# levia-than/neptune-pde-solver

Hardware: AMD Instinct MI355X
Metric: stencil-cell-updates/s (higher is better)
Workload: dtype f64

## Files before the change

### neptune-pde-solver_amd/csrc/kernels/apply_march.hpp

```cpp
#pragma once
#include "apply_common.hpp"

namespace neptune_hip {

struct InView {
  int64_t plane_b;
  int32_t row_b;
  int32_t sh[3];
  int32_t lo[3], hi[3];
  int32_t fix_k, fix_d;
};

template <class T, int NIN>
struct MarchParams {
  const T* in[NIN];
  T* out;
  int32_t N0, N1, N2;
  InView view[NIN];
  int32_t Ks, Kl;
  int32_t plb[3], pub[3];
  int64_t olb[3];
  int32_t rI0, rI1;
  int32_t rJ0, rJ1;
  int32_t chunk;
  uint32_t nJ, nK;
};

template <class T, int NIN>
__device__ __forceinline__ uint32_t view_row_bytes(const MarchParams<T, NIN>& P, int n, int32_t j) {
  if (NIN > 1 && n > 0) {
    const InView& vw = P.view[n];
    j = j < vw.lo[1] ? vw.lo[1] : (j > vw.hi[1] ? vw.hi[1] : j);
    return (uint32_t)(j + vw.sh[1]) * (uint32_t)vw.row_b + (uint32_t)vw.sh[2] * (uint32_t)sizeof(T);
  }
  j = j < 0 ? 0 : (j >= P.N1 ? P.N1 - 1 : j);
  return (uint32_t)j * (uint32_t)P.N2 * (uint32_t)sizeof(T);
}
template <class T, int NIN>
__device__ __forceinline__ uint32_t view_cell_bytes(const MarchParams<T, NIN>& P, int n, int32_t k) {
  if (NIN > 1 && n > 0) {
    const InView& vw = P.view[n];
    k = k < vw.lo[2] ? vw.lo[2] : (k > vw.hi[2] ? vw.hi[2] : k);
  } else {
    k = k < 0 ? 0 : (k >= P.N2 ? P.N2 - 1 : k);
  }
  return (uint32_t)k * (uint32_t)sizeof(T);
}
template <class T, int NIN>
__device__ __forceinline__ uint32_t view_lane_bytes(const MarchParams<T, NIN>& P, int n, int32_t k) {
  constexpr int VK = 16 / (int)sizeof(T);
  int32_t kmax = P.Kl;
  if (NIN > 1 && n > 0) kmax = P.view[n].hi[2] - VK + 1;
  return (uint32_t)(k < kmax ? k : kmax) * (uint32_t)sizeof(T);
}
template <class T, int NIN>
__device__ __forceinline__ const char* view_plane_base(const MarchParams<T, NIN>& P, int n, int32_t ip) {
  if (NIN > 1 && n > 0) {
    const InView& vw = P.view[n];
    const int32_t ic = ip < vw.lo[0] ? vw.lo[0] : (ip > vw.hi[0] ? vw.hi[0] : ip);
    return reinterpret_cast<const char*>(P.in[n]) + (int64_t)(ic + vw.sh[0]) * vw.plane_b;
  }
  const int32_t ic = ip < 0 ? 0 : (ip >= P.N0 ? P.N0 - 1 : ip);
  return reinterpret_cast<const char*>(P.in[n]) + (int64_t)ic * ((int64_t)P.N1 * P.N2 * (int64_t)sizeof(T));
}

template <class T> struct Vec16;
template <> struct Vec16<double> { typedef double type __attribute__((ext_vector_type(2))); };
template <> struct Vec16<float> { typedef float type __attribute__((ext_vector_type(4))); };

template <class T>
__device__ __forceinline__ typename Vec16<T>::type view_fix(typename Vec16<T>::type v, bool star, int32_t d) {
  if (d != 0) {
    if constexpr (sizeof(T) == 8) {
      v[0] = star ? v[1] : v[0];
    } else {
      if (d & 1) { const bool c = star; typename Vec16<T>::type w = v; v[0] = c ? w[1] : w[0]; v[1] = c ? w[2] : w[1]; v[2] = c ? w[3] : w[2]; }
      if (d & 2) { const bool c = star; typename Vec16<T>::type w = v; v[0] = c ? w[2] : w[0]; v[1] = c ? w[3] : w[1]; }
    }
  }
  return v;
}
template <class T, int NIN>
__device__ __forceinline__ int32_t view_fix_d(const MarchParams<T, NIN>& P, int n) { return (NIN > 1 && n > 0) ? P.view[n].fix_d : 0; }
template <class T, int NIN>
__device__ __forceinline__ bool view_fix_star(const MarchParams<T, NIN>& P, int n, int32_t k) { return NIN > 1 && n > 0 && k == P.view[n].fix_k; }

template <bool DPP>
__device__ __forceinline__ int shift32_from_prev(int x, int edge, int lane) {
  if constexpr (DPP) {
    return __builtin_amdgcn_update_dpp(edge, x, 0x138, 0xf, 0xf, false);
  } else {
    const int s = __shfl_up(x, 1);
    return lane == 0 ? edge : s;
  }
}
template <bool DPP>
__device__ __forceinline__ int shift32_from_next(int x, int edge, int lane) {
  if constexpr (DPP) {
    return __builtin_amdgcn_update_dpp(edge, x, 0x130, 0xf, 0xf, false);
  } else {
    const int s = __shfl_down(x, 1);
    return lane == kWave - 1 ? edge : s;
  }
}
template <bool DPP>
__device__ __forceinline__ float from_prev(float x, float edge, int lane) {
  return __int_as_float(shift32_from_prev<DPP>(__float_as_int(x), __float_as_int(edge), lane));
}
template <bool DPP>
__device__ __forceinline__ float from_next(float x, float edge, int lane) {
  return __int_as_float(shift32_from_next<DPP>(__float_as_int(x), __float_as_int(edge), lane));
}
template <bool DPP>
__device__ __forceinline__ double from_prev(double x, double edge, int lane) {
  const int lo = shift32_from_prev<DPP>(__double2loint(x), __double2loint(edge), lane);
  const int hi = shift32_from_prev<DPP>(__double2hiint(x), __double2hiint(edge), lane);
  return __hiloint2double(hi, lo);
}
template <bool DPP>
__device__ __forceinline__ double from_next(double x, double edge, int lane) {
  const int lo = shift32_from_next<DPP>(__double2loint(x), __double2loint(edge), lane);
  const int hi = shift32_from_next<DPP>(__double2hiint(x), __double2hiint(edge), lane);
  return __hiloint2double(hi, lo);
}

template <class T>
__device__ __forceinline__ T scalar_load(const T* p) {
  typedef const __attribute__((address_space(4))) T* cptr;
  return *(cptr)(p);
}

template <class T, int RANK, int NIN, class FP, int RJ, int r, int e, bool JK = false>
struct MarchAcc {
  static constexpr int VK = 16 / sizeof(T);
  static constexpr int R0 = JK ? 0 : FP::R0, R1 = JK ? FP::R0 : FP::R1, R2 = FP::R2;
  static constexpr unsigned HMASK = FP::HALO_MASK;
  static constexpr int NH = popcount_u(HMASK), NHX = NH ? NH : 1;
  static constexpr int NP = 2 * R0 + 1, NR = RJ + 2 * R1, NS = R2 ? R2 : 1;
  static constexpr int NPH = FP::BOX ? NP : 1;
  using V = typename Vec16<T>::type;

  const V (&ring)[NHX][NP][NR];
  const T (&lft)[NHX][NPH][NR][NS];
  const T (&rgt)[NHX][NPH][NR][NS];
  const V (&pt)[NIN][RJ];
  int64_t li, lj, lk;

  template <int IN, int... O>
  __device__ __forceinline__ T get() const {
    static_assert(IN >= 0 && IN < NIN, "input index out of range");
    constexpr int oi = JK ? 0 : PickOffset<RANK, AxisMap<RANK>::I, O...>::value;
    constexpr int oj = JK ? PickOffset<RANK, 0, O...>::value : PickOffset<RANK, AxisMap<RANK>::J, O...>::value;
    constexpr int ok = PickOffset<RANK, AxisMap<RANK>::K, O...>::value;
    if constexpr ((HMASK >> IN) & 1u) {
      constexpr int h = halo_slot(HMASK, IN);
      static_assert(oi >= -R0 && oi <= R0 && oj >= -R1 && oj <= R1 && ok >= -R2 && ok <= R2,
                    "access outside the declared footprint");
      static_assert(FP::BOX || ((oi != 0) + (oj != 0) + (ok != 0) <= 1),
                    "star footprint declared but a diagonal access is used");
      constexpr int p = oi + R0, s = r + R1 + oj, ke = e + ok;
      constexpr int ph = FP::BOX ? p : 0;
      if constexpr (ke < 0) return lft[h][ph][s][R2 + ke];
      else if constexpr (ke >= VK) return rgt[h][ph][s][ke - VK];
      else return ring[h][p][s][ke];
    } else {
      static_assert(oi == 0 && oj == 0 && ok == 0, "only halo inputs may be read at an offset");
      return pt[IN][r][e];
    }
  }
  template <int D>
  __device__ __forceinline__ int64_t idx() const {
    static_assert(D >= 0 && D < RANK, "index argument out of range");
    if constexpr (RANK == 3) return D == 0 ? li : (D == 1 ? lj : lk);
    else if constexpr (RANK == 2) return D == 0 ? (JK ? lj : li) : lk;
    else return lk;
  }
};

template <int RJ_, int WJ_, int WK_, bool DPP_, bool NT_, int PF_, bool NTL_, bool LDSJ_ = false, bool JK2_ = false,
          bool JHL_ = false, int KD_ = 1, bool PLN_ = false>
struct Tile {
  static constexpr int RJ = RJ_, WJ = WJ_, WK = WK_, PF = PF_, KD = KD_;
  static constexpr bool DPP = DPP_, NT = NT_, NTL = NTL_, LDSJ = LDSJ_, JK2 = JK2_, JHL = JHL_, PLN = PLN_;
};

template <class Body, class T, int RANK, int NIN, class FP, class TL>
__global__ __launch_bounds__(kWave* TL::WJ* TL::WK) void neptune_apply_march(MarchParams<T, NIN> P, Body body) {
  constexpr int RJ = TL::RJ, WJ = TL::WJ, WK = TL::WK, PF = TL::PF;
  constexpr bool DPP = TL::DPP, NT = TL::NT, NTL = TL::NTL;
  static_assert(PF >= 1, "prefetch distance");
  static_assert(FP::R2 <= 2 * (16 / (int)sizeof(T)), "K neighbours come from at most two lanes away");
  using V = typename Vec16<T>::type;
  constexpr int VK = 16 / sizeof(T);
  constexpr bool JK = RANK == 2 && TL::JK2;
  constexpr int R0 = JK ? 0 : FP::R0, R1 = JK ? FP::R0 : FP::R1, R2 = FP::R2;
  constexpr unsigned HMASK = FP::HALO_MASK;
  constexpr int NH = popcount_u(HMASK), NHX = NH ? NH : 1;
  constexpr bool BOX = FP::BOX;
  constexpr bool HAS_HALO = NH > 0;
  constexpr int NP = 2 * R0 + 1, NR = RJ + 2 * R1, NS = R2 ? R2 : 1;
  constexpr int NPH = BOX ? NP : 1;
  constexpr int HLEAD = BOX ? R0 : 0;
  constexpr int KD = (BOX || !HAS_HALO || R2 == 0 || JK) ? 1 : TL::KD;
  static_assert(KD >= 1 && KD <= 3, "K halo lead");
  constexpr int U = (PF % KD == 0) ? PF : (KD % PF == 0 ? KD : PF * KD);
  constexpr bool JH_LATE = TL::JHL && !BOX && R1 > 0;
  constexpr int PJ = JH_LATE ? R0 : NP - 1;
  constexpr int NJH = R1 > 0 ? 2 * R1 : 1;
  static_assert(HAS_HALO || (R0 == 0 && R1 == 0 && R2 == 0), "pointwise footprint must have zero radii");
  constexpr bool LDS_ALL = R1 > RJ;
  constexpr int LPUB = LDS_ALL ? RJ : 2 * R1;
  constexpr bool LDSJ = TL::LDSJ && WJ > 1 && R1 > 0 && HAS_HALO &&
                        2 * NHX * WJ * WK * LPUB * kWave * (int)sizeof(V) <= 64 * 1024;
  constexpr int LROWS = LDSJ ? LPUB : 1;
  auto halo_dist = [](int x) constexpr { return x < R1 ? (R1 - x + RJ - 1) / RJ : (x - R1) / RJ + 1; };
  auto halo_row = [](int x) constexpr { return x < R1 ? RJ * ((R1 - x + RJ - 1) / RJ) - (R1 - x) : (x - R1) % RJ; };
  __shared__ V lds_rows[LDSJ ? 2 : 1][LDSJ ? NHX : 1][LDSJ ? WJ * WK : 1][LROWS][LDSJ ? kWave : 1];

  const int lane = threadIdx.x & (kWave - 1);
  const int w = __builtin_amdgcn_readfirstlane(threadIdx.x >> 6);
  const int wj = w / WK, wk = w % WK;

  const uint32_t v = xcd_remap(blockIdx.x, gridDim.x);
  const uint32_t kt = v % P.nK;
  const uint32_t t = v / P.nK;
  const uint32_t jt = t % P.nJ;
  const uint32_t ct = t / P.nJ;

  const int32_t j0 = P.rJ0 + (int32_t)(jt * (WJ * RJ)) + wj * RJ;
  const int32_t kw = (int32_t)((kt * WK + wk) * (uint32_t)(kWave * VK));
  const int32_t k0 = kw + lane * VK;
  const bool lane_ok = k0 < P.Ks;
  const uint32_t lane_b = (uint32_t)(k0 < P.Kl ? k0 : P.Kl) * (uint32_t)sizeof(T);
  const int32_t kw_end = kw + kWave * VK;
  uint32_t lane_bv[NIN > 1 ? NIN : 1];
  int32_t fixd[NIN > 1 ? NIN : 1];
  bool fixs[NIN > 1 ? NIN : 1];
  static_for<(NIN > 1 ? NIN : 1)>([&](auto nc) {
    constexpr int n = nc;
    lane_bv[n] = view_lane_bytes(P, n, k0);
    fixd[n] = view_fix_d(P, n);
    fixs[n] = view_fix_star(P, n, k0);
  });

  const int32_t ib = P.rI0 + (int32_t)ct * P.chunk;
  const int32_t ie = (ib + P.chunk < P.rI1) ? ib + P.chunk : P.rI1;
  if (ib >= ie) {
    if constexpr (IsMonitored<Body>::value) { if (threadIdx.x == 0) body.partials[blockIdx.x] = (T)0; }
    return;
  }
  const int64_t plane_b = (int64_t)P.N1 * P.N2 * (int64_t)sizeof(T);
  [[maybe_unused]] T mon_acc = (T)0;

  constexpr int NV = NIN > 1 ? NIN : 1;
  uint32_t rowb[NV][NR];
  static_for<NV>([&](auto nc) {
    constexpr int n = nc;
    static_for<NR>([&](auto sc) {
      constexpr int s = sc;
      int32_t j = j0 + (s - R1);
      if constexpr (NIN > 1 && n > 0) {
        const InView& vw = P.view[n];
        j = j < vw.lo[1] ? vw.lo[1] : (j > vw.hi[1] ? vw.hi[1] : j);
        rowb[n][s] = (uint32_t)(j + vw.sh[1]) * (uint32_t)vw.row_b + (uint32_t)vw.sh[2] * (uint32_t)sizeof(T);
      } else {
        j = j < 0 ? 0 : (j >= P.N1 ? P.N1 - 1 : j);
        rowb[n][s] = (uint32_t)j * (uint32_t)P.N2 * (uint32_t)sizeof(T);
      }
    });
  });
  uint32_t khlb[NV][NS], khrb[NV][NS];
  static_for<NV>([&](auto nc) {
    constexpr int n = nc;
    static_for<NS>([&](auto xc) {
      constexpr int x = xc;
      int32_t kl = kw - R2 + x, kr = kw_end + x;
// ... 340 lines not shown
```

### neptune-pde-solver_amd/csrc/kernels/apply_march2.hpp

```cpp
#pragma once
#include "apply_march.hpp"

namespace neptune_hip {

template <class T, int NIN>
struct March2Params {
  const T* in[NIN];
  T* out;
  int32_t N0, N1, N2;
  int32_t plb[3], pub[3];
  int64_t olb[3];
  int32_t rI0, rI1;
  int32_t chunk;
  uint32_t nJ, nK;
};

template <class T, class FP, int NS>
struct March2Geom {
  static constexpr int VK = 16 / (int)sizeof(T), G = 64 / (int)sizeof(T);
  static constexpr int R0 = FP::R0, R1 = FP::R1, R2 = FP::R2;
  static constexpr int HG = G / 2 > VK ? G / 2 : VK;
  static constexpr int MK = (NS * R2 + HG - 1) / HG * HG;
  static constexpr int SPAN = kWave * VK, KEEPK = SPAN - 2 * MK;
  static constexpr int MJ = NS * R1;
  static constexpr int WARM = 2 * R0 * (NS - 1);
};

template <class T, int NIN>
struct Leapfrog2Params : March2Params<T, NIN> {
  T* out_v;
};

template <class Body, class T, int NIN, class FP, int NS, int RJ, int WJ, int MINW, bool LF = false>
__global__ __launch_bounds__(kWave* WJ, MINW) void neptune_apply_march2(
    std::conditional_t<LF, Leapfrog2Params<T, NIN>, March2Params<T, NIN>> P, Body body) {
  using V = typename Vec16<T>::type;
  using GM = March2Geom<T, FP, NS>;
  constexpr int VK = GM::VK, R0 = GM::R0, R1 = GM::R1, R2 = GM::R2, NP = 2 * R0 + 1;
  static_assert(NS >= 2 && NS <= 3, "two or three applies per pass");
  static_assert(!LF || (NS == 2 && NIN >= 2), "leapfrog: two stages, input 1 = the previous state");
  constexpr int TJ = RJ * WJ;
  constexpr int MK = GM::MK, SPAN = GM::SPAN;
  static_assert(R0 >= 1 && R0 <= 2 && R1 >= 1 && R1 <= 2 && R2 >= 1 && R2 <= 2 && !FP::BOX && FP::HALO_MASK == 1u, "star of input 0, radius 1..2");
  static_assert(RJ >= R1 && R2 <= VK && TJ > 2 * GM::MJ, "window too small for the footprint");
  constexpr int NQ = (NS - 1) * R0 + 1;
  constexpr int NF = NIN > 1 ? NIN - 1 : 1;
  __shared__ V lds[2][WJ][NS][2 * R1][kWave];

  const int lane = threadIdx.x & (kWave - 1);
  const int w = __builtin_amdgcn_readfirstlane(threadIdx.x >> 6);
  const uint32_t vb = xcd_remap(blockIdx.x, gridDim.x);
  const uint32_t kt = vb % P.nK;
  const uint32_t t = vb / P.nK;
  const uint32_t jt = t % P.nJ;
  const uint32_t ct = t / P.nJ;

  const int32_t Jb = (int32_t)(jt * (TJ - 2 * GM::MJ)) - GM::MJ;
  const int32_t j0 = Jb + w * RJ;
  const int32_t kw = (int32_t)(kt * GM::KEEPK) - MK;
  const int32_t k0 = kw + lane * VK;
  const int32_t kc = k0 < 0 ? 0 : (k0 > P.N2 - VK ? P.N2 - VK : k0);
  const uint32_t lane_b = (uint32_t)kc * (uint32_t)sizeof(T);
  uint32_t rowb[RJ];
  static_for<RJ>([&](auto rc) {
    constexpr int r = rc;
    int32_t j = j0 + r;
    j = j < 0 ? 0 : (j >= P.N1 ? P.N1 - 1 : j);
    rowb[r] = (uint32_t)j * (uint32_t)P.N2 * (uint32_t)sizeof(T);
  });
  const int64_t plane_b = (int64_t)P.N1 * P.N2 * (int64_t)sizeof(T);

  const int32_t ib = P.rI0 + (int32_t)ct * P.chunk;
  const int32_t ie = (ib + P.chunk < P.rI1) ? ib + P.chunk : P.rI1;
  if (ib >= ie) return;

  auto load_plane = [&](const T* field, int32_t ip, V(&rows)[RJ]) {
    const int32_t ic = ip < 0 ? 0 : (ip >= P.N0 ? P.N0 - 1 : ip);
    const char* base = reinterpret_cast<const char*>(field) + (int64_t)ic * plane_b;
    static_for<RJ>([&](auto rc) {
      constexpr int r = rc;
      rows[r] = *reinterpret_cast<const V*>(base + (rowb[r] + lane_b));
    });
  };

  bool row_keep[RJ], in_j[RJ], in_k[VK];
  static_for<RJ>([&](auto rc) {
    constexpr int r = rc;
    const int32_t j = j0 + r;
    row_keep[r] = j >= Jb + GM::MJ && j < Jb + TJ - GM::MJ && j >= 0 && j < P.N1;
    in_j[r] = j >= P.plb[1] && j < P.pub[1];
  });
  static_for<VK>([&](auto ec) {
    constexpr int e = ec;
    in_k[e] = (k0 + e) >= P.plb[2] && (k0 + e) < P.pub[2];
  });
  const bool lane_keep = k0 >= kw + MK && k0 < kw + SPAN - MK && k0 >= 0 && k0 < P.N2;

  auto stage = [&](const V(&pl)[NP][RJ], const V(&above)[R1], const V(&below)[R1], const V(&fx)[NF][NQ][RJ], const V(&xp)[RJ],
                   auto qc, int32_t ip, V(&res)[RJ]) {
    constexpr int q = decltype(qc)::value;
    V ring[1][NP][RJ + 2 * R1];
    T lft[1][1][RJ + 2 * R1][R2], rgt[1][1][RJ + 2 * R1][R2];
    V pt[NIN][RJ];
    static_for<RJ>([&](auto rc) {
      constexpr int r = rc;
      static_for<NP>([&](auto pc) { constexpr int pp = pc; ring[0][pp][r + R1] = pl[pp][r]; });
      static_for<R2>([&](auto xc) {
        constexpr int x = xc;
        constexpr int dl = R2 - x, dr = x + 1;
        lft[0][0][r + R1][x] = from_prev<true>(pl[R0][r][VK - dl], pl[R0][r][0], lane);
        rgt[0][0][r + R1][x] = from_next<true>(pl[R0][r][dr - 1], pl[R0][r][VK - 1], lane);
      });
      static_for<NIN>([&](auto nc) {
        constexpr int n = nc;
        if constexpr (LF && n == 1) pt[n][r] = xp[r];
        else if constexpr (n > 0) pt[n][r] = fx[n - 1][q][r];
      });
    });
    static_for<R1>([&](auto xc) {
      constexpr int x = xc;
      ring[0][R0][x] = above[x];
      ring[0][R0][RJ + R1 + x] = below[x];
    });
    const bool in_i = ip >= P.plb[0] && ip < P.pub[0];
    const int64_t li = (int64_t)ip + P.olb[0];
    static_for<RJ>([&](auto rc) {
      constexpr int r = rc;
      const int64_t lj = (int64_t)(j0 + r) + P.olb[1];
      static_for<VK>([&](auto ec) {
        constexpr int e = ec;
        const int64_t lk = (int64_t)(k0 + e) + P.olb[2];
        MarchAcc<T, 3, NIN, FP, RJ, r, e, false> acc{ring, lft, rgt, pt, li, lj, lk};
        const T val = body(acc);
        const T through = pl[R0][r][e];
        res[r][e] = (in_i && in_j[r] && in_k[e]) ? val : OutsideOf<Body, T>::apply(body, through);
      });
    });
  };

  V ring[NS][NP][RJ];
  V un[RJ];
  V fx[NF][NQ][RJ], fn[NF][RJ];
  V wres[RJ];
  const int32_t i0 = ib - GM::WARM;
  static_for<NP - 1>([&](auto pc) { constexpr int pp = pc; load_plane(P.in[0], i0 + NS * R0 - 2 * R0 + pp, ring[0][pp]); });
  load_plane(P.in[0], i0 + NS * R0, un);
  if constexpr (NIN > 1) {
    static_for<NIN - 1>([&](auto nc) {
      constexpr int n = nc;
      if constexpr (!(LF && n == 0))
        static_for<NQ - 1>([&](auto qc) { constexpr int q = qc; load_plane(P.in[n + 1], i0 + q, fx[n][q]); });
      load_plane(P.in[n + 1], i0 + NQ - 1, fn[n]);
    });
  }
  static_for<NS - 1>([&](auto kc) {
    constexpr int k = kc + 1;
    static_for<NP - 1>([&](auto pc) { constexpr int pp = pc; static_for<RJ>([&](auto rc) { constexpr int r = rc; ring[k][pp][r] = ring[0][0][r]; }); });
  });

  for (int32_t i = i0; i < ie; ++i) {
    static_for<RJ>([&](auto rc) { constexpr int r = rc; ring[0][NP - 1][r] = un[r]; });
    if constexpr (NIN > 1)
      static_for<NIN - 1>([&](auto nc) { constexpr int n = nc; static_for<RJ>([&](auto rc) { constexpr int r = rc; fx[n][NQ - 1][r] = fn[n][r]; }); });
    const int buf = (i - i0) & 1;
    static_for<NS>([&](auto kc) {
      constexpr int k = kc;
      static_for<R1>([&](auto xc) {
        constexpr int x = xc;
        lds[buf][w][k][x][lane] = ring[k][R0][x];
        lds[buf][w][k][R1 + x][lane] = ring[k][R0][RJ - R1 + x];
      });
    });
    __syncthreads();
    V above[NS][R1], below[NS][R1];
    static_for<NS>([&](auto kc) {
      constexpr int k = kc;
      static_for<R1>([&](auto xc) {
        constexpr int x = xc;
        above[k][x] = ring[k][R0][0];
        below[k][x] = ring[k][R0][RJ - 1];
        if (w > 0) above[k][x] = lds[buf][w - 1][k][R1 + x][lane];
        if (w < WJ - 1) below[k][x] = lds[buf][w + 1][k][x][lane];
      });
    });
    if (i + NS * R0 + 1 <= ie - 1 + NS * R0) {
      load_plane(P.in[0], i + NS * R0 + 1, un);
      if constexpr (NIN > 1) static_for<NIN - 1>([&](auto nc) { constexpr int n = nc; load_plane(P.in[n + 1], i + NQ, fn[n]); });
    }
    static_for<NS>([&](auto kc) {
      constexpr int k = kc;
      constexpr int q = (NS - k - 1) * R0;
      const V(&xp)[RJ] = (LF && k == 0) ? fx[0][NQ - 1] : ring[0][0];
      if constexpr (k + 1 < NS) stage(ring[k], above[k], below[k], fx, xp, std::integral_constant<int, q>{}, i + q, ring[k + 1][NP - 1]);
      else stage(ring[k], above[k], below[k], fx, xp, std::integral_constant<int, 0>{}, i, wres);
    });
    if (i >= ib && lane_keep) {
      char* obase = reinterpret_cast<char*>(P.out) + (int64_t)i * plane_b;
      static_for<RJ>([&](auto rc) {
        constexpr int r = rc;
        if (row_keep[r]) __builtin_nontemporal_store(wres[r], reinterpret_cast<V*>(obase + (rowb[r] + lane_b)));
      });
    }
    if constexpr (LF) {
      if (i + R0 >= ib && i + R0 < ie && lane_keep) {
        char* obase = reinterpret_cast<char*>(P.out_v) + (int64_t)(i + R0) * plane_b;
        static_for<RJ>([&](auto rc) {
          constexpr int r = rc;
          if (row_keep[r]) __builtin_nontemporal_store(ring[1][NP - 1][r], reinterpret_cast<V*>(obase + (rowb[r] + lane_b)));
        });
      }
    }
    static_for<NS>([&](auto kc) {
      constexpr int k = kc;
      static_for<NP - 1>([&](auto pc) { constexpr int pp = pc; static_for<RJ>([&](auto rc) { constexpr int r = rc; ring[k][pp][r] = ring[k][pp + 1][r]; }); });
    });
    if constexpr (NIN > 1)
      static_for<NIN - 1>([&](auto nc) {
        constexpr int n = nc;
        if constexpr (!(LF && n == 0))
          static_for<NQ - 1>([&](auto qc) { constexpr int q = qc; static_for<RJ>([&](auto rc) { constexpr int r = rc; fx[n][q][r] = fx[n][q + 1][r]; }); });
      });
  }
}


struct March2R2Params {
  const void* in[NEPTUNE_HIP_MAX_INPUTS];
  void* out;
  int32_t N0, N1;
  int32_t plb[2], pub[2];
  int64_t olb[2];
  int32_t rI0, rI1;
  int32_t chunk;
  uint32_t nK;
};

template <class FP>
constexpr bool march2_rank2_footprint() {
  return FP::MARCH_OK && !FP::BOX && FP::HALO_MASK == 1u && FP::R0 >= 1 && FP::R0 <= 2 && FP::R1 == 0 && FP::R2 >= 1 && FP::R2 <= 2;
}

struct Leapfrog2R2Params : March2R2Params {
  void* out_v;
};

template <class Body, class T, int NIN, class FP, int NS, int PF, bool LF = false>
__global__ __launch_bounds__(256) void neptune_apply_march2_rank2(std::conditional_t<LF, Leapfrog2R2Params, March2R2Params> P, Body body) {
  using V = typename Vec16<T>::type;
  using GM = March2Geom<T, FP, NS>;
  constexpr int VK = GM::VK, R0 = GM::R0, R2 = GM::R2, NP = 2 * R0 + 1, MK = GM::MK, SPAN = GM::SPAN, KEEPK = GM::KEEPK;
  static_assert(NS >= 2 && NS <= 3 && march2_rank2_footprint<FP>() && R2 <= VK, "window constants");
  static_assert(!LF || (NS == 2 && NIN >= 2), "leapfrog: two stages, input 1 = the previous state");
  constexpr int NQ = (NS - 1) * R0 + 1;
  constexpr int NF = NIN > 1 ? NIN - 1 : 1;
  const int lane = threadIdx.x & (kWave - 1);
  const uint32_t gw = blockIdx.x * (blockDim.x / kWave) + (threadIdx.x >> 6);
  const uint32_t kt = gw % P.nK, ct = gw / P.nK;
  const int32_t kw = (int32_t)(kt * KEEPK) - MK;
  const int32_t k0 = kw + lane * VK;
  const int32_t kc = k0 < 0 ? 0 : (k0 > P.N1 - VK ? P.N1 - VK : k0);
  const int32_t ib = P.rI0 + (int32_t)ct * P.chunk;
  const int32_t ie = (ib + P.chunk < P.rI1) ? ib + P.chunk : P.rI1;
  if (ib >= ie) return;
  T* out = static_cast<T*>(P.out);
  auto load_row = [&](int n, int32_t ip) -> V {
    const int32_t ic = ip < 0 ? 0 : (ip >= P.N0 ? P.N0 - 1 : ip);
    return *reinterpret_cast<const V*>(static_cast<const T*>(P.in[n]) + (int64_t)ic * P.N1 + kc);
  };
  bool in_k[VK];
  static_for<VK>([&](auto ec) { constexpr int e = ec; in_k[e] = (k0 + e) >= P.plb[1] && (k0 + e) < P.pub[1]; });
  const bool lane_keep = k0 >= kw + MK && k0 < kw + SPAN - MK && k0 >= 0 && k0 < P.N1;

  auto stage = [&](const V(&pl)[NP], const V(&fx)[NF][NQ], const V& xp, auto qc, int32_t ip) -> V {
    constexpr int q = decltype(qc)::value;
    V ring[1][NP][1];
    T lft[1][1][1][R2], rgt[1][1][1][R2];
    V pt[NIN][1];
    static_for<NP>([&](auto pc) { constexpr int pp = pc; ring[0][pp][0] = pl[pp]; });
    static_for<R2>([&](auto xc) {
      constexpr int x = xc;
      constexpr int dl = R2 - x, dr = x + 1;
      lft[0][0][0][x] = from_prev<true>(pl[R0][VK - dl], pl[R0][0], lane);
      rgt[0][0][0][x] = from_next<true>(pl[R0][dr - 1], pl[R0][VK - 1], lane);
    });
    static_for<NIN>([&](auto nc) {
      constexpr int n = nc;
      if constexpr (LF && n == 1) pt[n][0] = xp;
      else if constexpr (n > 0) pt[n][0] = fx[n - 1][q];
    });
    const bool in_i = ip >= P.plb[0] && ip < P.pub[0];
    const int64_t li = (int64_t)ip + P.olb[0];
    V res;
    static_for<VK>([&](auto ec) {
      constexpr int e = ec;
      const int64_t lk = (int64_t)(k0 + e) + P.olb[1];
      MarchAcc<T, 2, NIN, FP, 1, 0, e, false> acc{ring, lft, rgt, pt, li, 0, lk};
      const T val = body(acc);
      res[e] = (in_i && in_k[e]) ? val : OutsideOf<Body, T>::apply(body, pl[R0][e]);
    });
    return res;
  };

  V ring[NS][NP];
  V un[PF];
  V fx[NF][NQ], fn[NF][PF];
  const int32_t i0 = ib - GM::WARM;
  static_for<NP - 1>([&](auto pc) { constexpr int pp = pc; ring[0][pp] = load_row(0, i0 + NS * R0 - 2 * R0 + pp); });
  static_for<PF>([&](auto dc) { constexpr int d = dc; un[d] = load_row(0, i0 + NS * R0 + d); });
  if constexpr (NIN > 1) {
    static_for<NIN - 1>([&](auto nc) {
      constexpr int n = nc;
      if constexpr (!(LF && n == 0)) static_for<NQ - 1>([&](auto qc) { constexpr int q = qc; fx[n][q] = load_row(n + 1, i0 + q); });
      static_for<PF>([&](auto dc) { constexpr int d = dc; fn[n][d] = load_row(n + 1, i0 + NQ - 1 + d); });
    });
  }
  static_for<NS - 1>([&](auto kc2) { constexpr int k = kc2 + 1; static_for<NP - 1>([&](auto pc) { constexpr int pp = pc; ring[k][pp] = ring[0][0]; }); });
  auto step = [&](int32_t i, auto slot_c) {
    constexpr int slot = slot_c;
    ring[0][NP - 1] = un[slot];
    if constexpr (NIN > 1) static_for<NIN - 1>([&](auto nc) { constexpr int n = nc; fx[n][NQ - 1] = fn[n][slot]; });
    if (i + NS * R0 + PF <= ie - 1 + NS * R0) {
      un[slot] = load_row(0, i + NS * R0 + PF);
      if constexpr (NIN > 1) static_for<NIN - 1>([&](auto nc) { constexpr int n = nc; fn[n][slot] = load_row(n + 1, i + NQ - 1 + PF); });
    }
    V w;
    static_for<NS>([&](auto kc2) {
      constexpr int k = kc2;
      constexpr int q = (NS - k - 1) * R0;
      const V& xp = (LF && k == 0) ? fx[0][NQ - 1] : ring[0][0];
      if constexpr (k + 1 < NS) ring[k + 1][NP - 1] = stage(ring[k], fx, xp, std::integral_constant<int, q>{}, i + q);
      else w = stage(ring[k], fx, xp, std::integral_constant<int, 0>{}, i);
    });
    if (i >= ib && lane_keep) __builtin_nontemporal_store(w, reinterpret_cast<V*>(out + (int64_t)i * P.N1 + kc));
    if constexpr (LF) {
      if (i + R0 >= ib && i + R0 < ie && lane_keep)
        __builtin_nontemporal_store(ring[1][NP - 1], reinterpret_cast<V*>(static_cast<T*>(P.out_v) + (int64_t)(i + R0) * P.N1 + kc));
    }
    static_for<NS>([&](auto kc2) { constexpr int k = kc2; static_for<NP - 1>([&](auto pc) { constexpr int pp = pc; ring[k][pp] = ring[k][pp + 1]; }); });
    if constexpr (NIN > 1)
      static_for<NIN - 1>([&](auto nc) {
        constexpr int n = nc;
        if constexpr (!(LF && n == 0)) static_for<NQ - 1>([&](auto qc) { constexpr int q = qc; fx[n][q] = fx[n][q + 1]; });
      });
  };
  for (int32_t i = i0; i < ie; i += PF) {
    static_for<PF>([&](auto phc) {
      constexpr int ph = phc;
      if (i + ph < ie) step(i + ph, phc);
    });
  }
}


template <class T, int NIN, class FP>
inline bool march2_rank2_eligible(const neptune_hip_apply_geom_t* g, const void* const* in, const void* out) {
  constexpr int G = 64 / (int)sizeof(T);
  if (!g || g->rank != 2 || g->num_inputs != NIN) return false;
  if (!march2_rank2_footprint<FP>()) return false;
  int64_t n[2];
  const int r[2] = {FP::R0, FP::R2};
  for (int d = 0; d < 2; ++d) {
    n[d] = g->out_ub[d] - g->out_lb[d];
    for (int k = 0; k < NIN; ++k)
      if (g->in_lb[k][d] != g->out_lb[d] || g->in_ub[k][d] != g->out_ub[d]) return false;
    if (g->lb[d] < g->ub[d] && (g->lb[d] - r[d] < g->out_lb[d] || g->ub[d] + r[d] > g->out_ub[d])) return false;
  }
  if (g->region_lb[1] != 0 || g->region_ub[1] != n[1]) return false;
  if (n[1] % G != 0 || n[1] < 2 * G || n[0] < 1 || n[0] >= 0x7fffffffLL || n[1] >= 0x7fffffffLL) return false;
  if ((uintptr_t)out % 64 != 0) return false;
  for (int k = 0; k < NIN; ++k)
    if (!in[k] || (uintptr_t)in[k] % 64 != 0) return false;
  return true;
}

template <class Body, class T, int NIN, class FP, int NS, bool LF = false>
inline int launch_march2_rank2(const Body& body, const neptune_hip_apply_geom_t* g, const void* const* in, void* out, hipStream_t stream,
                               int chunk_req, void* out_v = nullptr) {
  if (!march2_rank2_eligible<T, NIN, FP>(g, in, out) || geom_bounds_empty(g)) return NEPTUNE_HIP_EUNSUPPORTED;
  constexpr int KEEPK = March2Geom<T, FP, NS>::KEEPK, PF = 4;
  std::conditional_t<LF, Leapfrog2R2Params, March2R2Params> P{};
  if constexpr (LF) P.out_v = out_v;
  for (int k = 0; k < NIN; ++k) P.in[k] = in[k];
  P.out = out;
  P.N0 = (int32_t)(g->out_ub[0] - g->out_lb[0]);
  P.N1 = (int32_t)(g->out_ub[1] - g->out_lb[1]);
  for (int d = 0; d < 2; ++d) {
    P.plb[d] = (int32_t)(g->lb[d] - g->out_lb[d]);
    P.pub[d] = (int32_t)(g->ub[d] - g->out_lb[d]);
    P.olb[d] = g->out_lb[d];
  }
  P.rI0 = (int32_t)g->region_lb[0];
  P.rI1 = (int32_t)g->region_ub[0];
  if (P.rI1 <= P.rI0) return NEPTUNE_HIP_OK;
  P.nK = (uint32_t)((P.N1 + KEEPK - 1) / KEEPK);
  const int64_t rows = P.rI1 - P.rI0;
  int64_t chunk = chunk_req > 0 ? chunk_req : 256;
  while (chunk_req <= 0 && chunk > 32 && (int64_t)P.nK * ((rows + chunk - 1) / chunk) < 8192) chunk /= 2;
  if (chunk > rows) chunk = rows;
  P.chunk = (int32_t)chunk;
  const int64_t waves = (int64_t)P.nK * ((rows + chunk - 1) / chunk);
  const int64_t blocks = (waves + 3) / 4;
  if (blocks <= 0 || blocks > 0x7fffffffLL) return NEPTUNE_HIP_EUNSUPPORTED;
  hipLaunchKernelGGL((neptune_apply_march2_rank2<Body, T, NIN, FP, NS, PF, LF>), dim3((uint32_t)blocks), dim3(256), 0, stream, P, body);
  NEPTUNE_HIP_CHECK(hipGetLastError());
  return NEPTUNE_HIP_OK;
}

template <class FP>
constexpr bool march2_footprint() {
  return FP::MARCH_OK && !FP::BOX && FP::HALO_MASK == 1u && FP::R0 >= 1 && FP::R0 <= 2 && FP::R1 >= 1 && FP::R1 <= 2 && FP::R2 >= 1 && FP::R2 <= 2;
}
template <class T, int NIN, class FP>
inline bool march2_eligible(const neptune_hip_apply_geom_t* g, const void* const* in, const void* out) {
  constexpr int G = 64 / (int)sizeof(T);
  if (!g || g->rank != 3 || g->num_inputs != NIN) return false;
  if (!march2_footprint<FP>()) return false;
  int64_t n[3];
  for (int d = 0; d < 3; ++d) {
    n[d] = g->out_ub[d] - g->out_lb[d];
    for (int k = 0; k < NIN; ++k)
      if (g->in_lb[k][d] != g->out_lb[d] || g->in_ub[k][d] != g->out_ub[d]) return false;
    if (d > 0 && (g->region_lb[d] != 0 || g->region_ub[d] != n[d])) return false;
  }
  if (n[2] % G != 0 || n[2] < 2 * G || n[1] < 8 || n[0] < 1) return false;
  if (n[1] * n[2] * (int64_t)sizeof(T) >= 0x7fffffffLL) return false;
  if ((uintptr_t)out % 64 != 0) return false;
  for (int k = 0; k < NIN; ++k)
    if (!in[k] || (uintptr_t)in[k] % 64 != 0) return false;
  const int r[3] = {FP::R0, FP::R1, FP::R2};
  for (int d = 0; d < 3; ++d)
    if (g->lb[d] < g->ub[d] && (g->lb[d] - r[d] < g->out_lb[d] || g->ub[d] + r[d] > g->out_ub[d])) return false;
  return true;
}

template <class Body, class T, int NIN, class FP, int NS, int RJ, int WJ, int MINW, bool LF = false>
inline int launch_march2_shape(const Body& body, const neptune_hip_apply_geom_t* g, const void* const* in, void* out, hipStream_t stream,
                               int chunk_req, void* out_v = nullptr) {
  using GM = March2Geom<T, FP, NS>;
  constexpr int KEEPJ = RJ * WJ - 2 * GM::MJ, KEEPK = GM::KEEPK;
  std::conditional_t<LF, Leapfrog2Params<T, NIN>, March2Params<T, NIN>> P{};
  if constexpr (LF) P.out_v = static_cast<T*>(out_v);
  for (int k = 0; k < NIN; ++k) P.in[k] = static_cast<const T*>(in[k]);
  P.out = static_cast<T*>(out);
  P.N0 = (int32_t)(g->out_ub[0] - g->out_lb[0]);
  P.N1 = (int32_t)(g->out_ub[1] - g->out_lb[1]);
  P.N2 = (int32_t)(g->out_ub[2] - g->out_lb[2]);
  for (int d = 0; d < 3; ++d) {
    P.plb[d] = (int32_t)(g->lb[d] - g->out_lb[d]);
    P.pub[d] = (int32_t)(g->ub[d] - g->out_lb[d]);
    P.olb[d] = g->out_lb[d];
  }
  P.rI0 = (int32_t)g->region_lb[0];
  P.rI1 = (int32_t)g->region_ub[0];
  if (P.rI1 <= P.rI0) return NEPTUNE_HIP_OK;
  P.nJ = (uint32_t)((P.N1 + KEEPJ - 1) / KEEPJ);
  P.nK = (uint32_t)((P.N2 + KEEPK - 1) / KEEPK);
  const int64_t planes = P.rI1 - P.rI0;
  int64_t chunk = chunk_req > 0 ? chunk_req : 128;
  while (chunk_req <= 0 && chunk > 16 && (int64_t)P.nJ * P.nK * ((planes + chunk - 1) / chunk) < 512) chunk /= 2;
  if (chunk > planes) chunk = planes;
  P.chunk = (int32_t)chunk;
  const int64_t blocks = (int64_t)P.nJ * P.nK * ((planes + chunk - 1) / chunk);
  if (blocks <= 0 || blocks > 0x7fffffffLL) return NEPTUNE_HIP_EUNSUPPORTED;
  hipLaunchKernelGGL((neptune_apply_march2<Body, T, NIN, FP, NS, RJ, WJ, MINW, LF>), dim3((uint32_t)blocks), dim3(kWave * WJ), 0, stream,
                     P, body);
  NEPTUNE_HIP_CHECK(hipGetLastError());
  return NEPTUNE_HIP_OK;
}

template <class Body, class T, int NIN, class FP, int NS>
inline int launch_march2(const Body& body, const neptune_hip_apply_geom_t* g, const void* const* in, void* out, hipStream_t stream,
                         int chunk_req) {
  if (!march2_eligible<T, NIN, FP>(g, in, out)) return NEPTUNE_HIP_EUNSUPPORTED;
  if (geom_bounds_empty(g)) return NEPTUNE_HIP_EUNSUPPORTED;
  static const int shape = [] { const char* e = getenv("NEPTUNE_HIP_MARCH2"); return e ? atoi(e) : 0; }();
  constexpr bool wide = FP::R0 > 1 || FP::R1 > 1 || FP::R2 > 1;
  if constexpr (wide) {
    if constexpr (NS != 2) {
      return NEPTUNE_HIP_EUNSUPPORTED;
    } else {
      switch (shape) {
        default:
        case 0: return launch_march2_shape<Body, T, NIN, FP, 2, 3, 8, 1>(body, g, in, out, stream, chunk_req);
        case 1: return launch_march2_shape<Body, T, NIN, FP, 2, 4, 8, 1>(body, g, in, out, stream, chunk_req);
      }
    }
  } else if constexpr (NS == 2) {
    switch (shape) {
      default:
      case 0: return launch_march2_shape<Body, T, NIN, FP, 2, 3, 16, 1>(body, g, in, out, stream, chunk_req);
#if NEPTUNE_HIP_FULL_VARIANTS
      case 1: return launch_march2_shape<Body, T, NIN, FP, 2, 7, 8, 1>(body, g, in, out, stream, chunk_req);
      case 2: return launch_march2_shape<Body, T, NIN, FP, 2, 4, 8, 1>(body, g, in, out, stream, chunk_req);
      case 3: return launch_march2_shape<Body, T, NIN, FP, 2, 2, 16, 1>(body, g, in, out, stream, chunk_req);
#endif
    }
  } else {
    switch (shape) {
      default:
      case 0: return launch_march2_shape<Body, T, NIN, FP, 3, 3, 12, 1>(body, g, in, out, stream, chunk_req);
#if NEPTUNE_HIP_FULL_VARIANTS
      case 1: return launch_march2_shape<Body, T, NIN, FP, 3, 2, 12, 1>(body, g, in, out, stream, chunk_req);
      case 2: return launch_march2_shape<Body, T, NIN, FP, 3, 4, 8, 1>(body, g, in, out, stream, chunk_req);
      case 3: return launch_march2_shape<Body, T, NIN, FP, 3, 5, 8, 1>(body, g, in, out, stream, chunk_req);
#endif
    }
  }
}

template <class Body, class T, int RANK, int NIN, class FP, int NS = 2>
inline int launch_apply_chain(const Body& body, const neptune_hip_apply_geom_t* g, const void* const* in, void* out,
                              hipStream_t stream, const neptune_hip_launch_cfg_t* cfg) {
  if constexpr (RANK == 3 && march2_footprint<FP>()) {
    if (!g || !in || !out) return NEPTUNE_HIP_EINVAL;
    for (int k = 0; k < NIN; ++k)
      if (!in[k]) return NEPTUNE_HIP_EINVAL;
    if (cfg && cfg->kernel == NEPTUNE_HIP_KERNEL_DIRECT) return NEPTUNE_HIP_EUNSUPPORTED;
    const int rc = geom_validate(g);
    if (rc != NEPTUNE_HIP_OK) return rc;
    return launch_march2<Body, T, NIN, FP, NS>(body, g, in, out, stream, cfg ? cfg->chunk : 0);
  } else if constexpr (RANK == 2 && march2_rank2_footprint<FP>()) {
    if (!g || !in || !out) return NEPTUNE_HIP_EINVAL;
    for (int k = 0; k < NIN; ++k)
      if (!in[k]) return NEPTUNE_HIP_EINVAL;
    if (cfg && cfg->kernel == NEPTUNE_HIP_KERNEL_DIRECT) return NEPTUNE_HIP_EUNSUPPORTED;
    const int rc = geom_validate(g);
    if (rc != NEPTUNE_HIP_OK) return rc;
    return launch_march2_rank2<Body, T, NIN, FP, NS>(body, g, in, out, stream, cfg ? cfg->chunk : 0);
  } else {
    return NEPTUNE_HIP_EUNSUPPORTED;
  }
}
template <class Body, class T, int RANK, int NIN, class FP>
inline int launch_apply_twice(const Body& body, const neptune_hip_apply_geom_t* g, const void* const* in, void* out,
                              hipStream_t stream, const neptune_hip_launch_cfg_t* cfg) {
  return launch_apply_chain<Body, T, RANK, NIN, FP, 2>(body, g, in, out, stream, cfg);
}
template <class Body, class T, int RANK, int NIN, class FP>
inline int launch_apply_thrice(const Body& body, const neptune_hip_apply_geom_t* g, const void* const* in, void* out,
                               hipStream_t stream, const neptune_hip_launch_cfg_t* cfg) {
  return launch_apply_chain<Body, T, RANK, NIN, FP, 3>(body, g, in, out, stream, cfg);
}

template <int RANK, int NIN, class FP>
constexpr bool leapfrog2_footprint() {
  if constexpr (RANK == 3) return march2_footprint<FP>() && NIN <= ((FP::R0 > 1 || FP::R1 > 1 || FP::R2 > 1) ? 2 : 3);
  else if constexpr (RANK == 2) return march2_rank2_footprint<FP>();
  else return false;
}
template <class T, int NIN>
inline bool leapfrog2_buffers_ok(const neptune_hip_apply_geom_t* g, const void* const* in, const void* out_v, const void* out_w) {
  if (!out_v || !out_w || (uintptr_t)out_v % 64 != 0) return false;
  const size_t bytes = geom_box_bytes(g->out_lb, g->out_ub, g->rank, sizeof(T));
  if (buffers_overlap(out_v, bytes, out_w, bytes)) return false;
  for (int k = 0; k < NIN; ++k)
    if (buffers_overlap(in[k], bytes, out_v, bytes) || buffers_overlap(in[k], bytes, out_w, bytes)) return false;
  return true;
}

template <class Body, class T, int RANK, int NIN, class FP>
inline int launch_apply_leapfrog2(const Body& body, const neptune_hip_apply_geom_t* g, const void* const* in, void* out_v, void* out_w,
                                  hipStream_t stream, const neptune_hip_launch_cfg_t* cfg) {
  static_assert(NIN >= 2, "a two-level scheme has the previous state as input 1");
  if constexpr (leapfrog2_footprint<RANK, NIN, FP>()) {
    if (!g || !in || !out_v || !out_w) return NEPTUNE_HIP_EINVAL;
    for (int k = 0; k < NIN; ++k)
      if (!in[k]) return NEPTUNE_HIP_EINVAL;
    if (cfg && (cfg->kernel == NEPTUNE_HIP_KERNEL_DIRECT || cfg->variant >= 0)) return NEPTUNE_HIP_EUNSUPPORTED;
    const int rc = geom_validate(g);
    if (rc != NEPTUNE_HIP_OK) return rc;
    if (g->num_inputs != NIN || !leapfrog2_buffers_ok<T, NIN>(g, in, out_v, out_w)) return NEPTUNE_HIP_EUNSUPPORTED;
    const int chunk = cfg ? cfg->chunk : 0;
    if constexpr (RANK == 3) {
      if (!march2_eligible<T, NIN, FP>(g, in, out_w) || geom_bounds_empty(g)) return NEPTUNE_HIP_EUNSUPPORTED;
      if constexpr (FP::R0 > 1 || FP::R1 > 1 || FP::R2 > 1)
        return launch_march2_shape<Body, T, NIN, FP, 2, 3, 8, 1, true>(body, g, in, out_w, stream, chunk, out_v);
      else if constexpr (NIN == 2)
        return launch_march2_shape<Body, T, NIN, FP, 2, 3, 12, 1, true>(body, g, in, out_w, stream, chunk, out_v);
      else
        return launch_march2_shape<Body, T, NIN, FP, 2, 4, 8, 1, true>(body, g, in, out_w, stream, chunk, out_v);
    } else {
      return launch_march2_rank2<Body, T, NIN, FP, 2, true>(body, g, in, out_w, stream, chunk, out_v);
    }
  } else {
    return NEPTUNE_HIP_EUNSUPPORTED;
  }
}

}
```

Baseline: 389.7 billion.

## Rotate march2 plane ring by unrolled phase, use buffer loads/stores and branchless masks

Restructures the march2 plane loop so the register ring of planes is indexed by a compile-time phase across an unrolled trip, instead of shifting every plane each iteration. It also adds an optional PF parameter for extra planes in flight. Global loads and stores move to raw buffer intrinsics, and stores are masked through the resource size and an out-of-range offset instead of branches. Other changes: edge-agnostic DPP lane shifts, neighbour reads taken from LDS unconditionally with clamped wave indices, and prefetches issued right after the first stage. The goal is to remove register moves, branches and address arithmetic per plane, at the cost of larger code from unrolling and correctness risks in the new masking and edge handling.

```diff
diff --git a/neptune-pde-solver_amd/csrc/kernels/apply_march.hpp b/neptune-pde-solver_amd/csrc/kernels/apply_march.hpp
--- a/neptune-pde-solver_amd/csrc/kernels/apply_march.hpp
+++ b/neptune-pde-solver_amd/csrc/kernels/apply_march.hpp
@@ -122,6 +122,17 @@
   const int lo = shift32_from_next<DPP>(__double2loint(x), __double2loint(edge), lane);
   const int hi = shift32_from_next<DPP>(__double2hiint(x), __double2hiint(edge), lane);
   return __hiloint2double(hi, lo);
+}
+
+__device__ __forceinline__ int shift32_from_prev_any_edge(int x) { return __builtin_amdgcn_mov_dpp(x, 0x138, 0xf, 0xf, true); }
+__device__ __forceinline__ int shift32_from_next_any_edge(int x) { return __builtin_amdgcn_mov_dpp(x, 0x130, 0xf, 0xf, true); }
+__device__ __forceinline__ float from_prev_any_edge(float x) { return __int_as_float(shift32_from_prev_any_edge(__float_as_int(x))); }
+__device__ __forceinline__ float from_next_any_edge(float x) { return __int_as_float(shift32_from_next_any_edge(__float_as_int(x))); }
+__device__ __forceinline__ double from_prev_any_edge(double x) {
+  return __hiloint2double(shift32_from_prev_any_edge(__double2hiint(x)), shift32_from_prev_any_edge(__double2loint(x)));
+}
+__device__ __forceinline__ double from_next_any_edge(double x) {
+  return __hiloint2double(shift32_from_next_any_edge(__double2hiint(x)), shift32_from_next_any_edge(__double2loint(x)));
 }
 
 template <class T>
diff --git a/neptune-pde-solver_amd/csrc/kernels/apply_march2.hpp b/neptune-pde-solver_amd/csrc/kernels/apply_march2.hpp
--- a/neptune-pde-solver_amd/csrc/kernels/apply_march2.hpp
+++ b/neptune-pde-solver_amd/csrc/kernels/apply_march2.hpp
@@ -31,12 +31,23 @@
   T* out_v;
 };
 
-template <class Body, class T, int NIN, class FP, int NS, int RJ, int WJ, int MINW, bool LF = false>
+constexpr int march2_gcd(int a, int b) { return b == 0 ? a : march2_gcd(b, a % b); }
+constexpr int march2_lcm(int a, int b) { return a / march2_gcd(a, b) * b; }
+
+template <class F, int... Ts>
+__device__ __forceinline__ bool march2_turn(F&& f, std::integer_sequence<int, Ts...>) {
+  return (f(std::integral_constant<int, Ts>{}) && ...);
+}
+
+template <class Body, class T, int NIN, class FP, int NS, int RJ, int WJ, int MINW, bool LF = false, int PF = 1>
 __global__ __launch_bounds__(kWave* WJ, MINW) void neptune_apply_march2(
     std::conditional_t<LF, Leapfrog2Params<T, NIN>, March2Params<T, NIN>> P, Body body) {
   using V = typename Vec16<T>::type;
   using GM = March2Geom<T, FP, NS>;
   constexpr int VK = GM::VK, R0 = GM::R0, R1 = GM::R1, R2 = GM::R2, NP = 2 * R0 + 1;
+  constexpr int N0S = NP + PF - 1;
+  constexpr int UNROLL = march2_lcm(march2_lcm(NP, N0S), PF);
+  static_assert(PF >= 1 && PF <= 3, "planes in flight per lane");
   static_assert(NS >= 2 && NS <= 3, "two or three applies per pass");
   static_assert(!LF || (NS == 2 && NIN >= 2), "leapfrog: two stages, input 1 = the previous state");
   constexpr int TJ = RJ * WJ;
@@ -74,20 +85,25 @@
   const int32_t ie = (ib + P.chunk < P.rI1) ? ib + P.chunk : P.rI1;
   if (ib >= ie) return;
 
+  typedef uint32_t U4 __attribute__((ext_vector_type(4)));
+  constexpr int kRsrcFlags = 0x00020000;
   auto load_plane = [&](const T* field, int32_t ip, V(&rows)[RJ]) {
     const int32_t ic = ip < 0 ? 0 : (ip >= P.N0 ? P.N0 - 1 : ip);
-    const char* base = reinterpret_cast<const char*>(field) + (int64_t)ic * plane_b;
+    char* base = const_cast<char*>(reinterpret_cast<const char*>(field)) + (int64_t)ic * plane_b;
+    const __amdgpu_buffer_rsrc_t rsrc = __builtin_amdgcn_make_buffer_rsrc(base, 0, (int32_t)plane_b, kRsrcFlags);
     static_for<RJ>([&](auto rc) {
       constexpr int r = rc;
-      rows[r] = *reinterpret_cast<const V*>(base + (rowb[r] + lane_b));
+      rows[r] = __builtin_bit_cast(V, __builtin_amdgcn_raw_buffer_load_b128(rsrc, (int32_t)lane_b, (int32_t)rowb[r], 0));
     });
   };
 
-  bool row_keep[RJ], in_j[RJ], in_k[VK];
+  auto less = [](int32_t a, int32_t b) -> int32_t { return (int32_t)((uint32_t)(a - b) >> 31); };
+  int32_t row_keep[RJ];
+  bool in_j[RJ], in_k[VK];
   static_for<RJ>([&](auto rc) {
     constexpr int r = rc;
     const int32_t j = j0 + r;
-    row_keep[r] = j >= Jb + GM::MJ && j < Jb + TJ - GM::MJ && j >= 0 && j < P.N1;
+    row_keep[r] = less(Jb + GM::MJ - 1, j) & less(j, Jb + TJ - GM::MJ) & less(-1, j) & less(j, P.N1);
     in_j[r] = j >= P.plb[1] && j < P.pub[1];
   });
   static_for<VK>([&](auto ec) {
@@ -95,21 +111,33 @@
     in_k[e] = (k0 + e) >= P.plb[2] && (k0 + e) < P.pub[2];
   });
   const bool lane_keep = k0 >= kw + MK && k0 < kw + SPAN - MK && k0 >= 0 && k0 < P.N2;
-
-  auto stage = [&](const V(&pl)[NP][RJ], const V(&above)[R1], const V(&below)[R1], const V(&fx)[NF][NQ][RJ], const V(&xp)[RJ],
-                   auto qc, int32_t ip, V(&res)[RJ]) {
-    constexpr int q = decltype(qc)::value;
+  const uint32_t store_voff = lane_keep ? lane_b : 0x80000000u;
+  int32_t row_bytes[RJ];
+  static_for<RJ>([&](auto rc) { constexpr int r = rc; row_bytes[r] = (int32_t)plane_b * row_keep[r]; });
+  auto store_plane = [&](T* field, int32_t ip, int32_t live, const V(&rows)[RJ]) {
+    char* obase = reinterpret_cast<char*>(field) + (int64_t)(ip * live) * plane_b;
+    static_for<RJ>([&](auto rc) {
+      constexpr int r = rc;
+      const __amdgpu_buffer_rsrc_t rsrc = __builtin_amdgcn_make_buffer_rsrc(obase, 0, row_bytes[r] * live, kRsrcFlags);
+      __builtin_amdgcn_raw_buffer_store_b128(__builtin_bit_cast(U4, rows[r]), rsrc, (int32_t)store_voff, (int32_t)rowb[r],  2);
+    });
+  };
+  auto stage = [&](const auto& slots, auto phc, const V(&above)[R1], const V(&below)[R1], const V(&fx)[NF][NQ][RJ],
+                   const V(&xp)[RJ], auto qc, int32_t ip, V(&res)[RJ]) {
+    constexpr int q = decltype(qc)::value, ph = decltype(phc)::value;
+    constexpr int NSL = (int)std::extent<std::remove_reference_t<decltype(slots)>>::value;
+    const V(&ctr)[RJ] = slots[(R0 + ph) % NSL];
     V ring[1][NP][RJ + 2 * R1];
     T lft[1][1][RJ + 2 * R1][R2], rgt[1][1][RJ + 2 * R1][R2];
     V pt[NIN][RJ];
     static_for<RJ>([&](auto rc) {
       constexpr int r = rc;
-      static_for<NP>([&](auto pc) { constexpr int pp = pc; ring[0][pp][r + R1] = pl[pp][r]; });
+      static_for<NP>([&](auto pc) { constexpr int pp = pc; ring[0][pp][r + R1] = slots[(pp + ph) % NSL][r]; });
       static_for<R2>([&](auto xc) {
         constexpr int x = xc;
         constexpr int dl = R2 - x, dr = x + 1;
-        lft[0][0][r + R1][x] = from_prev<true>(pl[R0][r][VK - dl], pl[R0][r][0], lane);
-        rgt[0][0][r + R1][x] = from_next<true>(pl[R0][r][dr - 1], pl[R0][r][VK - 1], lane);
+        lft[0][0][r + R1][x] = from_prev_any_edge(ctr[r][VK - dl]);
+        rgt[0][0][r + R1][x] = from_next_any_edge(ctr[r][dr - 1]);
       });
       static_for<NIN>([&](auto nc) {
         constexpr int n = nc;
@@ -132,95 +160,99 @@
         const int64_t lk = (int64_t)(k0 + e) + P.olb[2];
         MarchAcc<T, 3, NIN, FP, RJ, r, e, false> acc{ring, lft, rgt, pt, li, lj, lk};
         const T val = body(acc);
-        const T through = pl[R0][r][e];
+        const T through = ctr[r][e];
         res[r][e] = (in_i && in_j[r] && in_k[e]) ? val : OutsideOf<Body, T>::apply(body, through);
       });
     });
   };
 
+  V ring0[N0S][RJ];
   V ring[NS][NP][RJ];
-  V un[RJ];
-  V fx[NF][NQ][RJ], fn[NF][RJ];
+  V fx[NF][NQ][RJ], fn[NF][PF][RJ];
   V wres[RJ];
+  static_for<RJ>([&](auto rc) { constexpr int r = rc; wres[r] = V{}; });
   const int32_t i0 = ib - GM::WARM;
-  static_for<NP - 1>([&](auto pc) { constexpr int pp = pc; load_plane(P.in[0], i0 + NS * R0 - 2 * R0 + pp, ring[0][pp]); });
-  load_plane(P.in[0], i0 + NS * R0, un);
+  const int32_t last_u = ie - 1 + NS * R0;
+  const int32_t last_f = ie - 1 + NQ - 1;
+  static_for<N0S>([&](auto pc) { constexpr int pp = pc; load_plane(P.in[0], i0 + NS * R0 - 2 * R0 + pp, ring0[pp]); });
   if constexpr (NIN > 1) {
     static_for<NIN - 1>([&](auto nc) {
       constexpr int n = nc;
       if constexpr (!(LF && n == 0))
         static_for<NQ - 1>([&](auto qc) { constexpr int q = qc; load_plane(P.in[n + 1], i0 + q, fx[n][q]); });
-      load_plane(P.in[n + 1], i0 + NQ - 1, fn[n]);
+      static_for<PF>([&](auto dc) { constexpr int d = dc; load_plane(P.in[n + 1], i0 + NQ - 1 + d, fn[n][d]); });
     });
   }
   static_for<NS - 1>([&](auto kc) {
     constexpr int k = kc + 1;
-    static_for<NP - 1>([&](auto pc) { constexpr int pp = pc; static_for<RJ>([&](auto rc) { constexpr int r = rc; ring[k][pp][r] = ring[0][0][r]; }); });
+    static_for<NP - 1>([&](auto pc) { constexpr int pp = pc; static_for<RJ>([&](auto rc) { constexpr int r = rc; ring[k][pp][r] = ring0[0][r]; }); });
   });
 
-  for (int32_t i = i0; i < ie; ++i) {
-    static_for<RJ>([&](auto rc) { constexpr int r = rc; ring[0][NP - 1][r] = un[r]; });
+  const int wa = w > 0 ? w - 1 : w, wb = w < WJ - 1 ? w + 1 : w;
+  int32_t i = i0;
+  auto step = [&](auto tc) -> bool {
+    constexpr int t = decltype(tc)::value, ph = t % NP, p0 = t % N0S, us = t % PF;
+    constexpr int sC = (R0 + ph) % NP, sN = (NP - 1 + ph) % NP;
+    constexpr int sC0 = (R0 + p0) % N0S, sO0 = p0 % N0S;
     if constexpr (NIN > 1)
-      static_for<NIN - 1>([&](auto nc) { constexpr int n = nc; static_for<RJ>([&](auto rc) { constexpr int r = rc; fx[n][NQ - 1][r] = fn[n][r]; }); });
+      static_for<NIN - 1>([&](auto nc) { constexpr int n = nc; static_for<RJ>([&](auto rc) { constexpr int r = rc; fx[n][NQ - 1][r] = fn[n][us][r]; }); });
     const int buf = (i - i0) & 1;
     static_for<NS>([&](auto kc) {
       constexpr int k = kc;
+      const V(&ctr)[RJ] = k == 0 ? ring0[sC0] : ring[k][sC];
       static_for<R1>([&](auto xc) {
         constexpr int x = xc;
-        lds[buf][w][k][x][lane] = ring[k][R0][x];
-        lds[buf][w][k][R1 + x][lane] = ring[k][R0][RJ - R1 + x];
+        lds[buf][w][k][x][lane] = ctr[x];
+        lds[buf][w][k][R1 + x][lane] = ctr[RJ - R1 + x];
       });
     });
     __syncthreads();
-    V above[NS][R1], below[NS][R1];
-    static_for<NS>([&](auto kc) {
-      constexpr int k = kc;
-      static_for<R1>([&](auto xc) {
-        constexpr int x = xc;
-        above[k][x] = ring[k][R0][0];
-        below[k][x] = ring[k][R0][RJ - 1];
-        if (w > 0) above[k][x] = lds[buf][w - 1][k][R1 + x][lane];
-        if (w < WJ - 1) below[k][x] = lds[buf][w + 1][k][x][lane];
-      });
-    });
-    if (i + NS * R0 + 1 <= ie - 1 + NS * R0) {
-      load_plane(P.in[0], i + NS * R0 + 1, un);
-      if constexpr (NIN > 1) static_for<NIN - 1>([&](auto nc) { constexpr int n = nc; load_plane(P.in[n + 1], i + NQ, fn[n]); });
-    }
     static_for<NS>([&](auto kc) {
       constexpr int k = kc;
       constexpr int q = (NS - k - 1) * R0;
-      const V(&xp)[RJ] = (LF && k == 0) ? fx[0][NQ - 1] : ring[0][0];
-      if constexpr (k + 1 < NS) stage(ring[k], above[k], below[k], fx, xp, std::integral_constant<int, q>{}, i + q, ring[k + 1][NP - 1]);
-      else stage(ring[k], above[k], below[k], fx, xp, std::integral_constant<int, 0>{}, i, wres);
-    });
-    if (i >= ib && lane_keep) {
-      char* obase = reinterpret_cast<char*>(P.out) + (int64_t)i * plane_b;
-      static_for<RJ>([&](auto rc) {
-        constexpr int r = rc;
-        if (row_keep[r]) __builtin_nontemporal_store(wres[r], reinterpret_cast<V*>(obase + (rowb[r] + lane_b)));
+      const V(&xp)[RJ] = (LF && k == 0) ? fx[0][NQ - 1] : ring0[sO0];
+      V above[R1], below[R1];
+      static_for<R1>([&](auto xc) {
+        constexpr int x = xc;
+        above[x] = lds[buf][wa][k][R1 + x][lane];
+        below[x] = lds[buf][wb][k][x][lane];
       });
-    }
-    if constexpr (LF) {
-      if (i + R0 >= ib && i + R0 < ie && lane_keep) {
-        char* obase = reinterpret_cast<char*>(P.out_v) + (int64_t)(i + R0) * plane_b;
+      V(&res)[RJ] = k + 1 < NS ? ring[k + 1 < NS ? k + 1 : 0][sN] : wres;
+      {
+        V(&mine)[RJ] = k == 0 ? ring0[sC0] : ring[k][sC];
+        const T after = k == 0 ? wres[RJ - 1][VK - 1] : ring[k][sN][RJ - 1][VK - 1];
         static_for<RJ>([&](auto rc) {
           constexpr int r = rc;
-          if (row_keep[r]) __builtin_nontemporal_store(ring[1][NP - 1][r], reinterpret_cast<V*>(obase + (rowb[r] + lane_b)));
+          static_for<VK>([&](auto ec) {
+            constexpr int e = ec;
+            T c = mine[r][e];
+            asm volatile("" : "+v"(c) : "v"(after));
+            mine[r][e] = c;
+          });
         });
       }
+      if constexpr (k == 0) stage(ring0, std::integral_constant<int, p0>{}, above, below, fx, xp, std::integral_constant<int, q>{}, i + q, res);
+      else stage(ring[k], std::integral_constant<int, ph>{}, above, below, fx, xp, std::integral_constant<int, q>{}, i + q, res);
+      if constexpr (k == (LF ? NS - 1 : 0)) {
+        const int32_t ipu = i + NS * R0 + PF, ipf = i + NQ - 1 + PF;
+        load_plane(P.in[0], ipu < last_u ? ipu : last_u, ring0[sO0]);
+        if constexpr (NIN > 1)
+          static_for<NIN - 1>([&](auto nc) { constexpr int n = nc; load_plane(P.in[n + 1], ipf < last_f ? ipf : last_f, fn[n][us]); });
+      }
+    });
+    store_plane(P.out, i, less(ib - 1, i), wres);
+    if constexpr (LF) {
+      store_plane(P.out_v, i + R0, less(ib - 1, i + R0) & less(i + R0, ie), ring[1][sN]);
     }
-    static_for<NS>([&](auto kc) {
-      constexpr int k = kc;
-      static_for<NP - 1>([&](auto pc) { constexpr int pp = pc; static_for<RJ>([&](auto rc) { constexpr int r = rc; ring[k][pp][r] = ring[k][pp + 1][r]; }); });
-    });
     if constexpr (NIN > 1)
       static_for<NIN - 1>([&](auto nc) {
         constexpr int n = nc;
         if constexpr (!(LF && n == 0))
           static_for<NQ - 1>([&](auto qc) { constexpr int q = qc; static_for<RJ>([&](auto rc) { constexpr int r = rc; fx[n][q][r] = fx[n][q + 1][r]; }); });
       });
-  }
+    return ++i < ie;
+  };
+  while (march2_turn(step, std::make_integer_sequence<int, UNROLL>{})) {}
 }
 
 
@@ -433,7 +465,7 @@
   return true;
 }
 
-template <class Body, class T, int NIN, class FP, int NS, int RJ, int WJ, int MINW, bool LF = false>
+template <class Body, class T, int NIN, class FP, int NS, int RJ, int WJ, int MINW, bool LF = false, int PF = 1>
 inline int launch_march2_shape(const Body& body, const neptune_hip_apply_geom_t* g, const void* const* in, void* out, hipStream_t stream,
                                int chunk_req, void* out_v = nullptr) {
   using GM = March2Geom<T, FP, NS>;
@@ -462,7 +494,7 @@
   P.chunk = (int32_t)chunk;
   const int64_t blocks = (int64_t)P.nJ * P.nK * ((planes + chunk - 1) / chunk);
   if (blocks <= 0 || blocks > 0x7fffffffLL) return NEPTUNE_HIP_EUNSUPPORTED;
-  hipLaunchKernelGGL((neptune_apply_march2<Body, T, NIN, FP, NS, RJ, WJ, MINW, LF>), dim3((uint32_t)blocks), dim3(kWave * WJ), 0, stream,
+  hipLaunchKernelGGL((neptune_apply_march2<Body, T, NIN, FP, NS, RJ, WJ, MINW, LF, PF>), dim3((uint32_t)blocks), dim3(kWave * WJ), 0, stream,
                      P, body);
   NEPTUNE_HIP_CHECK(hipGetLastError());
   return NEPTUNE_HIP_OK;
@@ -493,6 +525,7 @@
       case 1: return launch_march2_shape<Body, T, NIN, FP, 2, 7, 8, 1>(body, g, in, out, stream, chunk_req);
       case 2: return launch_march2_shape<Body, T, NIN, FP, 2, 4, 8, 1>(body, g, in, out, stream, chunk_req);
       case 3: return launch_march2_shape<Body, T, NIN, FP, 2, 2, 16, 1>(body, g, in, out, stream, chunk_req);
+      case 4: return launch_march2_shape<Body, T, NIN, FP, 2, 3, 16, 1, false, 2>(body, g, in, out, stream, chunk_req);
 #endif
     }
   } else {
@@ -503,6 +536,7 @@
       case 1: return launch_march2_shape<Body, T, NIN, FP, 3, 2, 12, 1>(body, g, in, out, stream, chunk_req);
       case 2: return launch_march2_shape<Body, T, NIN, FP, 3, 4, 8, 1>(body, g, in, out, stream, chunk_req);
       case 3: return launch_march2_shape<Body, T, NIN, FP, 3, 5, 8, 1>(body, g, in, out, stream, chunk_req);
+      case 4: return launch_march2_shape<Body, T, NIN, FP, 3, 3, 12, 1, false, 2>(body, g, in, out, stream, chunk_req);
 #endif
     }
   }
```

After: 388.9 billion. No clear change (-0.2%).
